# diepthihoang/mpboot

Hardware: AMD Instinct MI355X
Metric: Fitch site-ops/sec (taxa x patterns x SPR-evals/s) (higher is better)
Workload: dtype u32

## Files before the change

### mpboot_amd/csrc/engine.cpp

```cpp
#include "engine.hpp"
#include <cstdlib>
#include "../host/simd_util.hpp"

#include <sched.h>

#include <algorithm>
#include <atomic>
#include <thread>
#include <ctime>
#include <chrono>
#include <climits>
#include <cstdio>
#include <cstring>

namespace mpf {

static_assert(sizeof(PlanOp) == sizeof(NvOp) && offsetof(PlanOp, pad) == offsetof(NvOp, pad), "refresh_stage sizes the ops as NvOp");

static inline double now_ms()
{
  return std::chrono::duration<double, std::milli>(std::chrono::steady_clock::now().time_since_epoch()).count();
}
struct ScopedMs {
  double &acc, t0;
// ... 450 lines not shown
{
  if (m <= 1 || tip(q)) return 1;
  if (m == vis_dense_m_ && visits_filled_epoch_ == topo_epoch_) return vis_dense_[(size_t)slot(q)];
  const size_t key = (size_t)q * 16 + (size_t)m;
  if (nvis_epoch_[key] == topo_epoch_) return nvis_val_[key];
  const int v = 1 + count_visits(back_[nx(q)], m - 1) + count_visits(back_[nx(nx(q))], m - 1);
  nvis_val_[key] = v;
  nvis_epoch_[key] = topo_epoch_;
  return v;
}

bool Engine::dev_sched_usable() const
{
  return have_tree_ && all_invalid_ && dev_sched_ && !sankoff_ && ntips_ == n_ && n_ >= 4 && g_.vw == 1 && g_.nv_pipe && views_mode_ >= 1 &&
         nslots_ <= kSchedMaxSlots;
}

int Engine::schedule_views_dev(int sweep_maxtrav)
{
  ScopedMs timer(stats.host_views_ms_total);
  RefreshShape s;
  s.nops = 3 * (size_t)(n_ - 2);
  s.maxlev = -1;
  const size_t n_prune = sweep_maxtrav > 0 ? 2 * (size_t)n_ - 2 : 0;
  if (kids_host_.size() != nslots_) kids_host_.assign(nslots_, make_uint2(0u, 0u));
  for (int v = n_ + 1; v <= 2 * n_ - 2; v++) {
    const int r0 = 3 * v;
    const uint32_t s0 = slot(back_[r0]), s1 = slot(back_[r0 + 1]), s2 = slot(back_[r0 + 2]);
    uint2 *k = &kids_host_[slot(r0)];
    k[0] = make_uint2(s1, s2);
    k[1] = make_uint2(s2, s0);
    k[2] = make_uint2(s0, s1);
  }
  kids_list_.clear();
  const size_t no_ride[2] = {0, 0};
  const RefreshStage sg = refresh_stage(nslots_, s.nops, (size_t)n_ + 2, n_prune, 64, 0, no_ride);
  HIPCHK(h_kstage_.reserve(sg.ops_off));
  HIPCHK(d_vstage_.reserve(sg.total));
  std::memcpy(h_kstage_.p, kids_host_.data(), sg.kids_bytes);
  uint8_t *src = d_vstage_.p;
  SweepDescArgs sw;
  if (n_prune) {
    uint32_t *np = reinterpret_cast<uint32_t *>(h_kstage_.p + sg.nodep_off);
    for (size_t i = 0; i < n_prune; i++) np[i] = slot(nodep_[i + 1]);
    const size_t cap = 8 * n_prune;
    HIPCHK(d_walk_.reserve(cap));
// ... 1 lines not shown
    HIPCHK(h_dsw_.reserve(4 + cap));
    HIPCHK(d_prog_.reserve(scan_prog_bytes((int)cap)));
    HIPCHK(reserve_results(cap * 63));
    sw.nodep = np;
    sw.n_prune = (uint32_t)n_prune;
    sw.maxtrav = (uint32_t)sweep_maxtrav;
    sw.split_cands = (uint32_t)std::max(0, split_cands_);
    sw.desc = d_walk_.p;
    sw.parts = d_parts_.p;
    sw.hdr_host = h_dsw_.p;
    sw.part_node = h_dsw_.p + 4;
    sw.hdr_dev = reinterpret_cast<uint32_t *>(src + sg.nlev_off) + 8;
    __atomic_store_n(h_dsw_.p + 3, 0u, __ATOMIC_RELAXED);
    __atomic_store_n(h_dsw_.p + 2, 0u, __ATOMIC_RELAXED);
    walk_gen_++;
    n_walk_ = 0;
    walk_out_ = 0;
    sweep_cache_valid_ = false;
    s.sw = &sw;
  }
  kids_dirty_ = false;
  kids_upload_ = false;
  kids_dev_ready_ = true;
  HIPCHK(launch_sched(st_, reinterpret_cast<const uint2 *>(h_kstage_.p), (uint32_t)n_, (uint32_t)s.nops, reinterpret_cast<NvOp *>(src + sg.ops_off),
                      reinterpret_cast<int32_t *>(src + sg.lev_off), reinterpret_cast<int32_t *>(src + sg.nlev_off), sw, reinterpret_cast<uint2 *>(src)));
  int rc = launch_refresh(src, sg, s);
  if (rc) return rc;
  const std::vector<int> &all = plan_.all;
  plan_.whole_tree(start_);
  upd_order_.resize(s.nops);
  size_t at = 0;
  if (all.size() != s.nops) { set_error("refresh schedule: the tree is not complete"); return MPF_E_STATE; }
  for (size_t i = all.size(); i >= 3; i -= 3) upd_order_[at++] = all[i - 3];
  for (size_t i = 0; i < all.size(); i += 3) { upd_order_[at++] = all[i + 1]; upd_order_[at++] = all[i + 2]; }
  rc = commit_refresh(sg, s, true, 2, true);
  if (n_prune) dsw_sched_gen_ = sched_gen_;
  return rc;
}

int Engine::launch_refresh(const uint8_t *src, const RefreshStage &sg, const RefreshShape &s)
{
  const NvOp *dops = reinterpret_cast<const NvOp *>(src + sg.ops_off);
  const int32_t *dlo = reinterpret_cast<const int32_t *>(src + sg.lev_off);
  HIPCHK(d_cntp_.reserve((size_t)std::max(tiles_for(g_), tiles_for_levels(g_)) * nslots_));
  if (timing_ >= 2) HIPCHK(hipEventRecord(ev2_, st_));
  RefreshExtra x;
  if (s.maxlev < 0) x.n_lev_ptr = reinterpret_cast<const int32_t *>(src + sg.nlev_off);
  x.wm_only = refresh_wm_only(s.chains);
  if (!x.wm_only) { const int rc = ensure_rows(); if (rc) return rc; }
  x.rows = rows_ok_;
  cnt_on_host_ = s.fold_inside && want_host_results_;
  if (cnt_on_host_) x.cnt_host = h_cnt();
  for (int i = 0; i < 2; i++) ride_[i].dev = sg.ride_off[i] ? src + sg.ride_off[i] : nullptr;
  const bool zero = s.ride && zero_req_ptr_;
  x.zero_ptr = zeroed_ptr_ = zero ? zero_req_ptr_ : nullptr;
  x.zero_words = (uint32_t)(zeroed_words_ = zero ? zero_req_words_ : 0);
  if (s.sw && plan_ride_) {
    x.wp_kids = reinterpret_cast<const uint2 *>(src);
    x.wp_n = (uint32_t)n_;
    x.wp_desc = d_walk_.p;
    x.wp_hdr = s.sw->hdr_dev;
    x.wp_prog = d_prog_.p;
    x.wp_out = d_out();
    x.wp_max_parts = 8 * s.sw->n_prune;
  }
  uint32_t *const vec = vec_base();
  uint32_t *const done = s.fold_inside ? d_done_.p : nullptr;
  if (s.chains) {
    if (s.direct) {
      x.kid_upd = reinterpret_cast<const uint32_t *>(src + sg.upd_off);
      x.n_kid_upd = (int)(plan_.kid_upd.size() / 3);
      x.kids = reinterpret_cast<uint2 *>(d_vstage_.p);
    }
    HIPCHK(launch_newview_chains(st_, g_, vec, dops, dlo, plan_.ch_levels, (int)s.nops, d_cntp_.p, (uint32_t)nslots_, d_cnt(), done, x));
    stats.view_launches++;
  } else if (views_mode_ >= 1) {
    if (s.generic && nv_waves_ > 0) x.waves_hint = nv_waves_;
    else if (s.generic && nv_waves_ == 0 && s.maxlev > 0 && g_.vw == 1 && g_.nv_pipe && !sankoff_) {
      const long per_level = ((long)s.nops + s.maxlev - 1) / s.maxlev;
      const long need = (2 * per_level * newview_tile(g_) + 63) / 64;
      x.waves_hint = need <= 2 ? 2 : need <= 4 ? 4 : need <= 8 ? 8 : 16;
    }
    HIPCHK(launch_newview_levels(st_, g_, vec, dops, dlo, s.maxlev < 0 ? 1 : s.maxlev, d_cntp_.p, (uint32_t)nslots_, d_cnt(), done, x));
    if (x.wm_only) rows_ok_ = false;
    stats.view_launches++;
  } else {
    const int32_t *lo = reinterpret_cast<const int32_t *>(h_vstage_.p + sg.lev_off);
    for (int l = 0; l < s.maxlev; l++) {
      HIPCHK(launch_newview(st_, g_, vec, dops + lo[l], lo[l + 1] - lo[l], d_cntp_.p, (uint32_t)nslots_));
      stats.view_launches++;
    }
  }
  if (!s.fold_inside)
    HIPCHK(launch_cntsum(st_, g_, dops, (int)s.nops, d_cntp_.p, (uint32_t)nslots_, d_cnt(),
                         (views_mode_ >= 1 && !s.chains) ? tiles_for_levels(g_) : 0));
  if (timing_ >= 2) { HIPCHK(hipEventRecord(ev3_, st_)); view_events_pending_ = true; }
  cnt_copy_pending_ = true;
  return MPF_OK;
}

int Engine::commit_refresh(const RefreshStage &sg, const RefreshShape &s, bool full, int made, bool cacheable)
{
  const bool both = views_mode_ >= 1 && !sankoff_ && g_.vw == 1 && g_.shoff != 0 && (s.chains || g_.nv_pipe);
  if (!both) shadow_ok_ = false;
  for (int r : upd_order_) valid_[r] = 1;
  all_invalid_ = false;
  if (full) { n_invalid_ = 0; views_valid_ = true; }
  else if (n_invalid_ > 0) {
    n_invalid_ -= (long)s.nops;
    if (n_invalid_ <= 0) {
      n_invalid_ = 0;
      views_valid_ = true;
      if (check_counts_)
        for (size_t r = 3 * ((size_t)n_ + 1); r < back_.size(); r++)
          if (back_[r] >= 0 && !valid_[r]) { set_error("view bookkeeping: invalid vector left behind"); return MPF_E_STATE; }
    }
  }
  pending_scores_ = true;
  if (made) {
    sched_cache_valid_ = (plan_cache_ & 2) && cacheable;
    sched_gen_++;
    sched_on_dev_ = made == 2;
    sc_stage_ = sg;
    if (sched_cache_valid_) { sc_maxlev_ = s.maxlev; sc_order_ = upd_order_; }
  }
  stats.newview_ops += s.nops;
  if (s.maxlev >= 0) dbg_levels_ += (uint64_t)(s.chains ? plan_.ch_levels : s.maxlev);
  stats.algorithmic_bytes += (uint64_t)s.nops * 3u * (uint64_t)g_.S * (uint64_t)Wref_ * 4u;
  return MPF_OK;
}

int Engine::schedule_views(const std::vector<int> *roots)
{
  if (!have_tree_) { set_error("no tree set"); return MPF_E_STATE; }
  ScopedMs timer(stats.host_views_ms_total);
  RefreshShape s;
  if (!roots && all_invalid_ && sched_cache_valid_ && !kids_dirty_ && !sankoff_) {
    s.nops = sc_order_.size();
    s.maxlev = sc_maxlev_;
    const int rc = launch_refresh(d_vstage_.p, sc_stage_, s);
    if (rc) return rc;
    upd_order_ = sc_order_;
    return commit_refresh(sc_stage_, s, true, 0, false);
  }
  if (!roots && dev_sched_usable()) return schedule_views_dev(0);
  const bool full = !roots;
  if (full) { plan_.whole_tree(start_); roots = &plan_.all; }
  const bool from_scratch = full && all_invalid_;
  plan_.close(*roots, from_scratch);
  if (kids_host_.size() != nslots_) kids_host_.assign(nslots_, make_uint2(0u, 0u));
  s.generic = true;
  const size_t nops = s.nops = plan_.order.size();
  s.maxlev = plan_.maxlev;
  s.chains = views_mode_ == 2 && !sankoff_ && nops > 0 && (long)nops <= chain_max_ops_ && g_.S * g_.vw <= 8;
  s.direct = s.chains && kids_dev_ready_ && (kids_dirty_ ? roots->size() + nops : kids_list_.size()) <= 4096;
  s.fold_inside = views_mode_ >= 1 && !sankoff_ && nops <= 512;
  s.ride = !sankoff_ && nops > 0 && views_mode_ >= 1;
  const auto slot_of = [this](int r) { return slot(r); };
  if (plan_.topo_delta(reinterpret_cast<uint32_t *>(kids_host_.data()), kids_list_, kids_dirty_, *roots, full, s.direct, slot_of))
// ... 759 lines not shown
    dsw_valid_ = false;
    rc = schedule_views_dev(mt);
  }
  if (rc) return rc;
  ScopedMs timer(stats.host_scan_ms_total);
  if (!warm) {
    if (!wait_host_flag(h_dsw_.p + 3)) HIPCHK(hipStreamSynchronize(st_));
    dsw_parts_ = h_dsw_.p[0];
    dsw_out_ = h_dsw_.p[1];
    dsw_walk_gen_ = walk_gen_;
    std::copy(key, key + 4, dsw_key_);
    dsw_valid_ = true;
  }
  const size_t nd = dsw_parts_, nout = dsw_out_;
  uint32_t best = UINT_MAX;
  if (nd > 0) {
    HIPCHK(d_ncand_.reserve(nd));
    HIPCHK(reserve_results(nout));
    HIPCHK(d_prog_.reserve(scan_prog_bytes((int)nd)));
    HIPCHK(h_pmin_.reserve(nd + 1));
    if (warm) HIPCHK(hipMemsetAsync(d_out(), 0, clear_words(nout) * sizeof(uint32_t), st_));
    if (timing_) HIPCHK(hipEventRecord(ev0_, st_));
    if (!warm) {
      if (!plan_ride_) HIPCHK(launch_walk_plan(st_, d_kids(), n_, d_walk_.p, (int)nd, d_prog_.p, d_out(), (uint32_t)clear_words(nout)));
      prog_gen_ = walk_gen_;
      parts_gen_ = walk_gen_;
      n_parts_dev_ = nd;
    }
    const bool wm = shadow_ok_ && scan_shadow_ && scan_prog_word_major(g_);
    HIPCHK(launch_scan_prog(st_, g_, wm ? vec_base() : vec_rows(), d_walk_.p, (int)nd, d_prog_.p, d_out(), d_ncand_.p, nullptr, (uint32_t)nout, d_done_.p + 8, nullptr,
                            wm));
    stats.plan_launches++;
    if (timing_) HIPCHK(hipEventRecord(ev1_, st_));
    __atomic_store_n(h_pmin_.p + nd, 0u, __ATOMIC_RELAXED);
    HIPCHK(launch_part_min(st_, d_out(), d_parts_.p, (int)nd, h_pmin_.p, d_cnt(), cnt_copy_pending_ ? h_cnt() : nullptr, (uint32_t)nslots_,
                           d_done_.p + 24));
    cnt_copy_pending_ = false;
    if (!wait_host_flag(h_pmin_.p + nd)) HIPCHK(hipStreamSynchronize(st_));
    float ms = 0;
    if (timing_ && hipEventElapsedTime(&ms, ev0_, ev1_) == hipSuccess) { stats.last_scan_kernel_ms = ms; stats.scan_kernel_ms_total += ms; }
    if (plan_event_pending_) {
      if (hipEventElapsedTime(&ms, ev4_, ev0_) == hipSuccess) stats.plan_kernel_ms_total += ms;
      plan_event_pending_ = false;
    }
    stats.scan_launches++;
  } else {
    if (cnt_copy_pending_) {
// ... 132 lines not shown
  long sum = 0;
  int site = 0;
  for (int k = 0; k < P_ && site < n_sites; k++) {
    if (first_site_[(size_t)k] < 0) continue;
    for (int w = 0; w < wgt_[(size_t)k] && site < n_sites; w++) { site_pars[site++] = ptn[(size_t)k]; sum += ptn[(size_t)k]; }
  }
  for (; site < n_sites; site++) site_pars[site] = 0;
  if (total) *total = (int32_t)sum;
  return MPF_OK;
}

int Engine::set_option(const std::string &key, int64_t v)
{
  if (key == "scan_batch") { if (v < 1) return MPF_E_INVALID; scan_batch_ = (int)v; return MPF_OK; }
  if (key == "words_per_lane") {
    if (sankoff_ && v != 1) { set_error("words_per_lane: weighted mode uses one pattern per lane"); return MPF_E_INVALID; }
    if (!(v == 1 || v == 2 || v == 4) || (g_.S == 20 && v == 4)) { set_error("words_per_lane: 1|2|4 (protein: 1|2)"); return MPF_E_INVALID; }
    if (g_.S >= 20) return MPF_OK;
    g_.vw = (int)v;
    return MPF_OK;
  }
  if (key == "dev_sched") { dev_sched_ = v != 0; sched_cache_valid_ = false; dsw_valid_ = false; return MPF_OK; }
  if (key == "dev_plan") { dev_plan_ = v != 0; plan_ride_ = !(v & 2); dsw_valid_ = false; return MPF_OK; }
  if (key == "refresh_wm") { refresh_wm_ = v != 0; return MPF_OK; }
  if (key == "scan_shadow") { scan_shadow_ = v != 0; return MPF_OK; }
  if (key == "reduce") { g_.reduce = v ? 1 : 0; return MPF_OK; }
  if (key == "xcd_map") { g_.map = v ? 1 : 0; return MPF_OK; }
  if (key == "scan_mode") { scan_mode_ = v ? 1 : 0; return MPF_OK; }
  if (key == "views_pipe") { g_.nv_pipe = v != 0; sched_cache_valid_ = false; return MPF_OK; }
  if (key == "views_tile") {
    if (v != 32 && v != 16 && v != 8 && v != 4 && v != 0) { set_error("views_tile: 32, 16, 8 or 4 words (0: chosen from the row length)"); return MPF_E_INVALID; }
    g_.nv_tile = (int)v;
    sched_cache_valid_ = false;
    return MPF_OK;
  }
  if (key == "views_mode") { views_mode_ = v < 0 ? 0 : v > 2 ? 2 : (int)v; sched_cache_valid_ = false; return MPF_OK; }
  if (key == "host_poll") { host_poll_ = v ? 1 : 0; return MPF_OK; }
  if (key == "ufb_fast") { ufb_fast_ = v ? 1 : 0; return MPF_OK; }
  if (key == "ufb_quiet") { ufb_quiet_ = v ? 1 : 0; return MPF_OK; }
  if (key == "deep_scratch_kwords") {
    if (v < 1 || v > (1 << 22)) { set_error("deep_scratch_kwords: 1 .. 4194304"); return MPF_E_INVALID; }
    deep_scratch_words_ = (size_t)v << 10; d_deep_.release(); g_.deep_scratch = nullptr; g_.deep_scratch_words = 0;
    return MPF_OK;
  }
  if (key == "grow_device") { grow_device_ = v ? 1 : 0; return MPF_OK; }
  if (key == "grow_tile") { if (v != 0 && v != 1 && v != 2 && v != 4 && v != 8 && v != -1) { set_error("grow_tile: 0 (word-major copy where there is one, else fitted), -1 (fitted quad tiles), 1, 2, 4 or 8"); return MPF_E_INVALID; } grow_vw_ = (int)v; return MPF_OK; }
// ... 60 lines not shown
  return MPF_E_INVALID;
}

int Engine::scan_trace(uint64_t *out, uint64_t cap, uint64_t *n)
{
  if (climb_trace_) {
    *n = cd_.h_trace.size() / 2;
    if (cap >= *n && *n) std::memcpy(out, cd_.h_trace.data(), cd_.h_trace.size() * sizeof(uint32_t));
    return MPF_OK;
  }
  *n = trace_words_;
  if (!trace_words_ || cap < trace_words_) return MPF_OK;
  activate();
  HIPCHK(hipMemcpy(out, d_trace_.p, trace_words_ * sizeof(unsigned long long), hipMemcpyDeviceToHost));
  return MPF_OK;
}

int Engine::get_option(const std::string &key, int64_t *v) const
{
  if (key == "scan_prog") *v = scan_prog_;
  else if (key == "prog_min_descs") *v = prog_min_descs_;
  else if (key == "refresh_wm") *v = refresh_wm_ ? 1 : 0;
  else if (key == "refresh_wm_active") *v = (refresh_wm_ && !sankoff_ && g_.S == 4 && g_.shoff != 0) ? 1 : 0;
  else if (key == "rows_ok") *v = rows_ok_ ? 1 : 0;
  else if (key == "ensure_rows_launches") *v = (int64_t)ensure_rows_launches_;
  else if (key == "scan_batch") *v = scan_batch_;
  else if (key == "words_per_lane") *v = g_.vw;
  else if (key == "kernel_states") *v = g_.S;
  else if (key == "reduce") *v = g_.reduce;
  else if (key == "xcd_map") *v = g_.map;
  else if (key == "scan_mode") *v = scan_mode_;
  else if (key == "views_mode") *v = views_mode_;
  else if (key == "views_pipe") *v = g_.nv_pipe;
  else if (key == "views_tile") *v = g_.nv_tile;
  else if (key == "plan_cache") *v = plan_cache_;
  else if (key == "sched_levels" || key == "sched_ticks" || key == "sched_desc_ticks") {
    int32_t w[16] = {0};
    if (sched_on_dev_ && d_vstage_.p) { (void)hipStreamSynchronize(st_); (void)hipMemcpy(w, d_vstage_.p + sc_stage_.nlev_off, 64, hipMemcpyDeviceToHost); }
    *v = w[key == "sched_levels" ? 0 : key == "sched_ticks" ? 1 : 2];
  }
  else if (key == "split_below") *v = split_below_;
  else if (key == "split_cands") *v = split_cands_;
  else if (key == "chain_max_ops") *v = chain_max_ops_;
  else if (key == "timing") *v = timing_;
  else if (key == "ufb_fast") *v = ufb_fast_;
  else if (key == "ufb_quiet") *v = ufb_quiet_;
// ... 80 lines not shown
```

### mpboot_amd/csrc/engine.hpp

```cpp
#pragma once
#include <hip/hip_runtime.h>

#include <algorithm>
#include <cmath>
#include <chrono>
#include <cstdint>
#include <functional>
#include <map>
#include <unordered_map>
#include <memory>
#include <climits>
#include <set>
#include <string>
#include <utility>
#include <vector>

#include "../../include/mpfitch.h"
#include "../host/rng.hpp"
#include "../host/ufb_books.hpp"
#include "../host/list_tree.hpp"
#include "../host/split_sets.hpp"
#include "../host/refresh_plan.hpp"
#include "../host/many_shape.hpp"
#include "climb.hpp"
// ... 202 lines not shown
  int P() const { return P_; }
  int S() const { return sref_; }
  int Wref() const { return Wref_; }
  int Wp() const { return g_.Wp; }
  int n_informative() const { return ninf_; }
  const std::vector<int32_t> &informative() const { return inf_; }

  int set_tree(const int32_t *back);
  void get_tree(int32_t *back) const;
  void reset_node_order();
  void node_rectifier();

  int score_tree(uint32_t *score);
  int pattern_scores(uint16_t *ptn, int32_t *total);
  int site_scores(int32_t *site_pars, int n_sites, int32_t *total);
  int update_views();
  int tree_length(uint32_t *len);
  void invalidate_all();
  void invalidate_vectors();
  void invalidate_node(int node);
  int schedule_views(const std::vector<int> *roots);
  bool dev_sched_usable() const;
  int schedule_views_dev(int sweep_maxtrav);
  struct RefreshShape { size_t nops = 0; int maxlev = 0; bool chains = false, direct = false, fold_inside = false, generic = false, ride = false;
                        const SweepDescArgs *sw = nullptr; };
  int launch_refresh(const uint8_t *src, const RefreshStage &sg, const RefreshShape &s);
  int commit_refresh(const RefreshStage &sg, const RefreshShape &s, bool full, int made, bool cacheable);
  int sweep_scan_dev(int maxtrav, uint64_t *n_tests, uint32_t *min_mp);
  void finish_views();
  void collect_scan_roots(int p, int mintrav, int maxtrav, std::vector<int> &roots) const;

  int plan_scan(int rec, int mintrav, int maxtrav, ScanPlan &plan);
  int run_scans(std::vector<ScanPlan> &plans, std::vector<uint32_t> &out_host);
  int plan_walk(int rec, int mintrav, int maxtrav, ScanPlan &plan, bool split);
  int run_walks(std::vector<ScanPlan> &plans, const uint32_t **out_host);
  int run_walks_finish(std::vector<ScanPlan> &plans, const uint32_t **out_host);
  static bool wait_host_flag(const uint32_t *flag);
  struct WaitScope { WaitScope(); ~WaitScope(); };
  static void wait_pause();
  int scan_batch(std::vector<ScanPlan> &plans, const int *recs, int count, int mintrav, int maxtrav, const uint32_t **out);
  int candidate_record(const ScanPlan &plan, size_t c);
  void enumerate_side(int x, int mintrav, int maxtrav, std::vector<int32_t> &q) const { enumerate_side(back_, x, mintrav, maxtrav, q); }
  void enumerate_side(const std::vector<int32_t> &bk, int x, int mintrav, int maxtrav, std::vector<int32_t> &q) const { books::enumerate_side(n_, bk, x, mintrav, maxtrav, q); }
  int spr_scan(int rec, int mintrav, int maxtrav, std::vector<int32_t> &q, std::vector<uint32_t> &mp, int &n_p);
  int sweep_scan(int mintrav, int maxtrav, uint64_t *n_tests, uint32_t *min_mp);
  int sweep_costs(int mintrav, int maxtrav, uint64_t cap, uint32_t *mp, uint64_t *offsets, uint64_t *n_tests);
  int node_order(int32_t *recs);
// ... 421 lines not shown
  int scan_mode_ = 1;
  int scan_prog_ = 1, prog_min_descs_ = 256;
  DevBuf<uint8_t> d_prog_;
  int plan_cache_ = 7;
  bool sched_cache_valid_ = false;
  RefreshStage sc_stage_ = {};
  int sc_maxlev_ = 0;
  bool dev_sched_ = true;
  bool dev_plan_ = true;
  PinBuf<uint8_t> h_kstage_;
  PinBuf<uint32_t> h_dsw_;
  bool dsw_valid_ = false;
  uint64_t dsw_walk_gen_ = 0;
  uint64_t sched_gen_ = 0, dsw_sched_gen_ = ~0ull;
  int dsw_key_[4] = {0, 0, 0, 0};
  uint32_t dsw_parts_ = 0, dsw_out_ = 0;
  bool sched_on_dev_ = false;
  bool shadow_ok_ = false;
  bool scan_shadow_ = true;
  bool rows_ok_ = true;
  bool refresh_wm_ = true;
  uint64_t ensure_rows_launches_ = 0;
  bool plan_ride_ = true;
  std::vector<int> sc_order_;
  bool sweep_cache_valid_ = false, walk_dev_reuse_ = false;
  uint64_t walk_gen_ = 0, sweep_cache_gen_ = 0;
  uint64_t prog_gen_ = ~0ull;
  size_t sweep_cache_nwalk_ = 0;
  uint32_t sweep_cache_out_ = 0;
  int sweep_cache_key_[6] = {0, 0, 0, 0, 0, 0};
  std::vector<int> sweep_cache_recs_;
  int scan_trace_ = 0;
  DevBuf<unsigned long long> d_trace_;
  size_t trace_words_ = 0;
  std::vector<uint32_t> out_scratch_;
  std::vector<ScanPlan> sweep_plans_;
  std::vector<uint32_t> sc_keep_mp_;
  std::vector<uint64_t> sc_keep_off_;
  uint64_t sc_keep_key_[4] = {0, 0, 0, 0}, pack_gen_ = 0;
  bool sc_keep_valid_ = false;
  std::vector<int32_t> nvis_val_, nvis_epoch_;
  int32_t topo_epoch_ = 1;
  int count_visits(int q, int m);
  void fill_visit_counts(int maxm);
  int32_t visits_filled_epoch_ = 0;
  std::vector<int32_t> vis_dense_, vis_a_;
// ... 50 lines not shown
```

### mpboot_amd/csrc/kernels.hip

```cpp
#include "kernels.hpp"
#include <cstdlib>

namespace mpf {


__device__ __forceinline__ uint32_t wave_sum_dpp(uint32_t v)
{
  v += (uint32_t)__builtin_amdgcn_update_dpp(0, (int)v, 0xB1, 0xF, 0xF, false);
  v += (uint32_t)__builtin_amdgcn_update_dpp(0, (int)v, 0x4E, 0xF, 0xF, false);
  v += (uint32_t)__builtin_amdgcn_update_dpp(0, (int)v, 0x141, 0xF, 0xF, false);
  v += (uint32_t)__builtin_amdgcn_update_dpp(0, (int)v, 0x140, 0xF, 0xF, false);
  v += (uint32_t)__builtin_amdgcn_update_dpp(0, (int)v, 0x142, 0xA, 0xF, false);
  v += (uint32_t)__builtin_amdgcn_update_dpp(0, (int)v, 0x143, 0xC, 0xF, false);
  return v;
}

template <int TW>
__device__ __forceinline__ uint32_t group_sum(uint32_t v)
{
  v += (uint32_t)__builtin_amdgcn_update_dpp(0, (int)v, 0xB1, 0xF, 0xF, false);
  v += (uint32_t)__builtin_amdgcn_update_dpp(0, (int)v, 0x4E, 0xF, 0xF, false);
  if constexpr (TW >= 8) v += (uint32_t)__builtin_amdgcn_update_dpp(0, (int)v, 0x141, 0xF, 0xF, false);
  if constexpr (TW >= 16) v += (uint32_t)__builtin_amdgcn_update_dpp(0, (int)v, 0x140, 0xF, 0xF, false);
  if constexpr (TW == 32) v += (uint32_t)__shfl_xor((int)v, 16, 32);
// ... 222 lines not shown
  const int w0 = lane_word<VW>(tile, lane, Wp, valid);
  Tile<S, VW> a, b, c;
  load_tile<S, VW>(a, vec, o.a, Wp, w0);
  load_tile<S, VW>(b, vec, o.b, Wp, w0);
  uint32_t cost = fitch<S, VW>(c, a, b);
  if (valid) store_tile<S, VW>(c, vec, o.dst, Wp, w0);
  cost = valid ? cost : 0u;
  const uint32_t tot = wave_total<RED>(cost);
  if (lane == 0) cntp[(size_t)tile * nslots + o.dst] = tot;
}

template <int S, int VW, int RED>
__global__ __launch_bounds__(256) void k_newview(uint32_t *__restrict__ vec, const NvOp *__restrict__ ops, int n_ops,
                                                 uint32_t *__restrict__ cntp, uint32_t nslots, int Wp, int tiles)
{
  const int lane = threadIdx.x & 63;
  int gw = blockIdx.x * (blockDim.x >> 6) + (threadIdx.x >> 6);
  gw = __builtin_amdgcn_readfirstlane(gw);
  if (gw >= n_ops * tiles) return;
  const int op = gw / tiles, tile = gw - op * tiles;
  newview_one<S, VW, RED>(vec, ops[op], cntp, nslots, Wp, tile, lane);
}

__device__ __forceinline__ void fold_counts(const NvOp *__restrict__ ops, int n_ops, const uint32_t *__restrict__ cntp,
                                            uint32_t nslots, int tiles, uint32_t *__restrict__ cnt, int tid, int nthreads,
                                            uint32_t *__restrict__ cnt_host = nullptr)
{
  const int l32 = tid & 31, grp = tid >> 5, ngrp = nthreads >> 5;
  for (int i = grp; i < n_ops; i += 2 * ngrp) {
    const int j = i + ngrp < n_ops ? i + ngrp : i;
    const uint32_t d0 = ops[i].dst, d1 = ops[j].dst;
    uint32_t s0 = 0, s1 = 0;
    for (int t = l32; t < tiles; t += 32) {
      s0 += __builtin_nontemporal_load(cntp + (size_t)t * nslots + d0);
      s1 += __builtin_nontemporal_load(cntp + (size_t)t * nslots + d1);
    }
#pragma unroll
    for (int m = 16; m >= 1; m >>= 1) {
      s0 += (uint32_t)__shfl_xor((int)s0, m, 32);
      s1 += (uint32_t)__shfl_xor((int)s1, m, 32);
    }
    if (l32 == 0) {
      cnt[d0] = s0;
      if (j != i) cnt[d1] = s1;
      if (cnt_host) {
        cnt_host[d0] = s0;
        if (j != i) cnt_host[d1] = s1;
      }
    }
  }
}

template <int S, int VW, int RED>
__global__ __launch_bounds__(1024) void k_newview_wg(uint32_t *__restrict__ vec, const NvOp *__restrict__ ops,
                                                     const int32_t *__restrict__ lev_off, int n_lev,
                                                     uint32_t *__restrict__ cntp, uint32_t nslots, int Wp,
                                                     uint32_t *__restrict__ cnt, uint32_t *__restrict__ done,
                                                     RefreshExtra x)
{
  __shared__ int s_last;
  const int lane = threadIdx.x & 63;
  const int wave = __builtin_amdgcn_readfirstlane((int)(threadIdx.x >> 6));
  const int nw = (int)(blockDim.x >> 6);
  const int tile = blockIdx.x;
  bool valid;
  const int w0 = lane_word<VW>(tile, lane, Wp, valid);
  for (uint32_t i = blockIdx.x * blockDim.x + threadIdx.x; i < x.zero_words; i += gridDim.x * blockDim.x) x.zero_ptr[i] = 0u;
  for (int l = 0; l < n_lev; l++) {
    const int b = lev_off[l], e = lev_off[l + 1];
    int i = b + wave;
    for (; i + nw < e; i += 2 * nw) {
      const NvOp o0 = ops[i], o1 = ops[i + nw];
      Tile<S, VW> a0, b0, a1, b1, c0, c1;
// ... 475 lines not shown
  if (per <= 2u) return launch(int_c<2>());
  if (per <= 3u) return launch(int_c<3>());
  if (per <= 4u) return launch(int_c<4>());
  if (per <= 6u) return launch(int_c<6>());
  if (per <= 8u) return launch(int_c<8>());
  return launch(int_c<16>());
}

__global__ __launch_bounds__(256) void k_cntsum(const NvOp *__restrict__ ops, int n_ops, const uint32_t *__restrict__ cntp, uint32_t nslots,
                                                int tiles, uint32_t *__restrict__ cnt, uint32_t *__restrict__ cnt_host)
{
  const int l32 = threadIdx.x & 31;
  const int i = (int)(blockIdx.x * (blockDim.x >> 5) + (threadIdx.x >> 5));
  if (i >= n_ops) return;
  const uint32_t dst = ops[i].dst;
  uint32_t s = 0;
  for (int t = l32; t < tiles; t += 32) s += cntp[(size_t)t * nslots + dst];
#pragma unroll
  for (int m = 16; m >= 1; m >>= 1) s += (uint32_t)__shfl_xor((int)s, m, 32);
  if (l32 == 0) {
    cnt[dst] = s;
    if (cnt_host) cnt_host[dst] = s;
  }
}


template <int S, int VW, int RED, bool WM = false>
__global__ __launch_bounds__(256) void k_evaluate(const uint32_t *__restrict__ vec, const EvOp *__restrict__ ops,
                                                  int n_ops, uint32_t *__restrict__ out, int Wp, int tiles)
{
  const int lane = threadIdx.x & 63;
  int gw = blockIdx.x * (blockDim.x >> 6) + (threadIdx.x >> 6);
  gw = __builtin_amdgcn_readfirstlane(gw);
  if (gw >= n_ops * tiles) return;
  const int op = gw / tiles, tile = gw - op * tiles;
  const EvOp o = ops[op];
  bool valid;
  const int w0 = lane_word<VW>(tile, lane, Wp, valid);
  Tile<S, VW> a, b;
  if constexpr (WM) {
    static_assert(S == 4 && VW == 1, "word-major copy: DNA, one word per lane");
    load_tile_wm(a, vec, o.a, Wp, w0);
    load_tile_wm(b, vec, o.b, Wp, w0);
  } else {
    load_tile<S, VW>(a, vec, o.a, Wp, w0);
    load_tile<S, VW>(b, vec, o.b, Wp, w0);
// ... 2088 lines not shown
```

### mpboot_amd/csrc/kernels.hpp

```cpp
#pragma once
#include <hip/hip_runtime.h>
#include <stdint.h>
#include <atomic>
#include <type_traits>

#include "../host/list_tree.hpp"

namespace mpf {

struct NvOp { uint32_t dst, a, b, pad; };

struct EvOp { uint32_t a, b, out, pad; };

struct ScanOp { uint32_t own, sib, meta, out; };
struct ScanHdr { uint32_t op_begin, op_end, s_slot, pad ; };

enum { SCAN_CHAIN = 0, SCAN_ROOT = 1, SCAN_JOIN = 2, SCAN_EVAL = 3 };

struct WalkDesc { uint32_t s_cid, xa_cid, xb_cid, trav ,
                  out_base, pad0, pad1, pad2; };
constexpr int kWalkMaxDepth = 8;
constexpr int kMaxDepth = 12;
constexpr int scan_reg_depth(int S, bool sankoff) { return sankoff ? (S != 4 ? 6 : kMaxDepth) : (S >= 32 ? 6 : kMaxDepth); }

// ... 79 lines not shown
                            const uint32_t *tip_slots);
hipError_t launch_newview(hipStream_t st, const Geometry &g, uint32_t *vec, const NvOp *ops, int n_ops, uint32_t *cntp,
                          uint32_t nslots);
struct RefreshExtra { const uint32_t *kid_upd = nullptr; int n_kid_upd = 0; uint2 *kids = nullptr; uint32_t *zero_ptr = nullptr; uint32_t zero_words = 0;
                      uint32_t *cnt_host = nullptr;
                      const int32_t *n_lev_ptr = nullptr;
                      const uint2 *wp_kids = nullptr; uint32_t wp_n = 0; const WalkDesc *wp_desc = nullptr; const uint32_t *wp_hdr = nullptr ;
                      void *wp_prog = nullptr; uint32_t *wp_out = nullptr; uint32_t wp_max_parts = 0;
                      uint32_t *shadow = nullptr;
                      int wm_only = 0, rows = 0;
                      int waves_hint = 0;  };
constexpr uint32_t kSchedMaxSlots = 16384;
struct SweepDescArgs {
  const uint32_t *nodep = nullptr;
  uint32_t n_prune = 0, maxtrav = 0, split_cands = 0;
  WalkDesc *desc = nullptr;
  uint2 *parts = nullptr;
  uint32_t *part_node = nullptr;
  uint32_t *hdr_host = nullptr;
  uint32_t *hdr_dev = nullptr;
};
hipError_t launch_sched(hipStream_t st, const uint2 *kids, uint32_t n_taxa, uint32_t n_ops, NvOp *ops, int32_t *lev_off, int32_t *n_lev,
                        const SweepDescArgs &sw = SweepDescArgs(), uint2 *kids_copy = nullptr);
hipError_t launch_newview_levels(hipStream_t st, const Geometry &g, uint32_t *vec, const NvOp *ops, const int32_t *lev_off,
                                 int n_lev, uint32_t *cntp, uint32_t nslots, uint32_t *cnt, uint32_t *done,
                                 const RefreshExtra &x = RefreshExtra());
hipError_t launch_newview_chains(hipStream_t st, const Geometry &g, uint32_t *vec, const NvOp *ops, const int32_t *wl_off,
                                 int n_lev, int n_ops, uint32_t *cntp, uint32_t nslots, uint32_t *cnt, uint32_t *done,
                                 const RefreshExtra &x);
hipError_t launch_part_min(hipStream_t st, const uint32_t *out, const uint2 *parts, int n_parts, uint32_t *pmin,
                           const uint32_t *cnt = nullptr, uint32_t *cnt_host = nullptr, uint32_t n_cnt = 0, uint32_t *done = nullptr);
hipError_t launch_cntsum(hipStream_t st, const Geometry &g, const NvOp *ops, int n_ops, const uint32_t *cntp,
                         uint32_t nslots, uint32_t *cnt, int tiles = 0 ,
                         uint32_t *cnt_host = nullptr );
int tiles_for(const Geometry &g);
int newview_tile(const Geometry &g);
int tiles_for_levels(const Geometry &g);
hipError_t launch_evaluate(hipStream_t st, const Geometry &g, const uint32_t *vec, const EvOp *ops, int n_ops,
                           uint32_t *out, bool word_major = false);
hipError_t launch_rows_from_wm(hipStream_t st, const Geometry &g, uint32_t *vec, const uint32_t *slots, int n_slots);
struct NniDesc { uint32_t a, b, c0, c1; };
hipError_t launch_nni_eval(hipStream_t st, const Geometry &g, const uint32_t *vec, const NniDesc *desc, int n_br,
                           unsigned long long *out, int vw, bool word_major);
hipError_t launch_nni_eval_masks(hipStream_t st, const Geometry &g, const uint32_t *vec, const NniDesc *desc, int n_br,
                                 unsigned long long *out, int vw, bool word_major, uint32_t *plane0, uint32_t *plane1);
hipError_t launch_snk_nni_eval(hipStream_t st, const Geometry &g, const uint32_t *vec, const NniDesc *desc, int n_br,
// ... 46 lines not shown
```

Baseline: 18080000 billion.

## Fuse level scheduling into the full-tree newview kernel for self-scheduled refresh

A new kernel builds the level lists itself. Each block derives the next level's ready ops in LDS while it computes Fitch for the current level, so the separate launch_sched kernel and the device ops/level arrays are no longer needed on the main path. A small kids-copy kernel replaces the scheduling launch. The count fold runs inside the kernel for small trees, and otherwise in a slot-indexed cntsum that can also carry the walk-plan work. Each block redundantly recomputes the schedule in 1024-thread blocks with large LDS, which may limit occupancy, and an optional extra block writes out the ops list for caching.

```diff
diff --git a/mpboot_amd/csrc/engine.cpp b/mpboot_amd/csrc/engine.cpp
--- a/mpboot_amd/csrc/engine.cpp
+++ b/mpboot_amd/csrc/engine.cpp
@@ -496,6 +496,9 @@
   RefreshShape s;
   s.nops = 3 * (size_t)(n_ - 2);
   s.maxlev = -1;
+  s.self = refresh_self_sched_ && newview_self_supported(g_, (uint32_t)n_, (uint32_t)s.nops);
+  s.fold_inside = s.self && s.nops <= 512;
+  self_active_ = s.self;
   const size_t n_prune = sweep_maxtrav > 0 ? 2 * (size_t)n_ - 2 : 0;
   if (kids_host_.size() != nslots_) kids_host_.assign(nslots_, make_uint2(0u, 0u));
   for (int v = n_ + 1; v <= 2 * n_ - 2; v++) {
@@ -543,8 +546,11 @@
   kids_dirty_ = false;
   kids_upload_ = false;
   kids_dev_ready_ = true;
-  HIPCHK(launch_sched(st_, reinterpret_cast<const uint2 *>(h_kstage_.p), (uint32_t)n_, (uint32_t)s.nops, reinterpret_cast<NvOp *>(src + sg.ops_off),
-                      reinterpret_cast<int32_t *>(src + sg.lev_off), reinterpret_cast<int32_t *>(src + sg.nlev_off), sw, reinterpret_cast<uint2 *>(src)));
+  if (s.self)
+    HIPCHK(launch_kids_copy(st_, reinterpret_cast<const uint2 *>(h_kstage_.p), reinterpret_cast<uint2 *>(src), (uint32_t)n_, (uint32_t)s.nops));
+  else
+    HIPCHK(launch_sched(st_, reinterpret_cast<const uint2 *>(h_kstage_.p), (uint32_t)n_, (uint32_t)s.nops, reinterpret_cast<NvOp *>(src + sg.ops_off),
+                        reinterpret_cast<int32_t *>(src + sg.lev_off), reinterpret_cast<int32_t *>(src + sg.nlev_off), sw, reinterpret_cast<uint2 *>(src)));
   int rc = launch_refresh(src, sg, s);
   if (rc) return rc;
   const std::vector<int> &all = plan_.all;
@@ -576,7 +582,8 @@
   const bool zero = s.ride && zero_req_ptr_;
   x.zero_ptr = zeroed_ptr_ = zero ? zero_req_ptr_ : nullptr;
   x.zero_words = (uint32_t)(zeroed_words_ = zero ? zero_req_words_ : 0);
-  if (s.sw && plan_ride_) {
+  plan_rode_ = s.sw && plan_ride_ && !(s.self && s.fold_inside);
+  if (plan_rode_) {
     x.wp_kids = reinterpret_cast<const uint2 *>(src);
     x.wp_n = (uint32_t)n_;
     x.wp_desc = d_walk_.p;
@@ -594,6 +601,14 @@
       x.kids = reinterpret_cast<uint2 *>(d_vstage_.p);
     }
     HIPCHK(launch_newview_chains(st_, g_, vec, dops, dlo, plan_.ch_levels, (int)s.nops, d_cntp_.p, (uint32_t)nslots_, d_cnt(), done, x));
+    stats.view_launches++;
+  } else if (s.self) {
+    HIPCHK(launch_newview_self(st_, g_, vec, reinterpret_cast<const uint2 *>(src), (uint32_t)n_, (uint32_t)s.nops, d_cntp_.p, (uint32_t)nslots_, d_cnt(), done,
+                               reinterpret_cast<int32_t *>(d_vstage_.p + sg.nlev_off), reinterpret_cast<const uint2 *>(h_kstage_.p),
+                               s.sw ? *s.sw : SweepDescArgs(), x,
+                               (plan_cache_ & 2) ? reinterpret_cast<NvOp *>(d_vstage_.p + sg.ops_off) : nullptr,
+                               (plan_cache_ & 2) ? reinterpret_cast<int32_t *>(d_vstage_.p + sg.lev_off) : nullptr));
+    if (x.wm_only) rows_ok_ = false;
     stats.view_launches++;
   } else if (views_mode_ >= 1) {
     if (s.generic && nv_waves_ > 0) x.waves_hint = nv_waves_;
@@ -612,7 +627,9 @@
       stats.view_launches++;
     }
   }
-  if (!s.fold_inside)
+  if (s.self) {
+    if (!s.fold_inside) HIPCHK(launch_cntsum_slots(st_, (uint32_t)n_, (int)s.nops, d_cntp_.p, (uint32_t)nslots_, d_cnt(), tiles_for_levels(g_), x));
+  } else if (!s.fold_inside)
     HIPCHK(launch_cntsum(st_, g_, dops, (int)s.nops, d_cntp_.p, (uint32_t)nslots_, d_cnt(),
                          (views_mode_ >= 1 && !s.chains) ? tiles_for_levels(g_) : 0));
   if (timing_ >= 2) { HIPCHK(hipEventRecord(ev3_, st_)); view_events_pending_ = true; }
@@ -656,6 +673,7 @@
   if (!have_tree_) { set_error("no tree set"); return MPF_E_STATE; }
   ScopedMs timer(stats.host_views_ms_total);
   RefreshShape s;
+  if (all_invalid_) self_active_ = false;
   if (!roots && all_invalid_ && sched_cache_valid_ && !kids_dirty_ && !sankoff_) {
     s.nops = sc_order_.size();
     s.maxlev = sc_maxlev_;
@@ -1461,7 +1479,7 @@
     if (warm) HIPCHK(hipMemsetAsync(d_out(), 0, clear_words(nout) * sizeof(uint32_t), st_));
     if (timing_) HIPCHK(hipEventRecord(ev0_, st_));
     if (!warm) {
-      if (!plan_ride_) HIPCHK(launch_walk_plan(st_, d_kids(), n_, d_walk_.p, (int)nd, d_prog_.p, d_out(), (uint32_t)clear_words(nout)));
+      if (!plan_rode_) HIPCHK(launch_walk_plan(st_, d_kids(), n_, d_walk_.p, (int)nd, d_prog_.p, d_out(), (uint32_t)clear_words(nout)));
       prog_gen_ = walk_gen_;
       parts_gen_ = walk_gen_;
       n_parts_dev_ = nd;
@@ -1640,6 +1658,7 @@
   }
   if (key == "dev_sched") { dev_sched_ = v != 0; sched_cache_valid_ = false; dsw_valid_ = false; return MPF_OK; }
   if (key == "dev_plan") { dev_plan_ = v != 0; plan_ride_ = !(v & 2); dsw_valid_ = false; return MPF_OK; }
+  if (key == "refresh_self_sched") { refresh_self_sched_ = v != 0; sched_cache_valid_ = false; dsw_valid_ = false; return MPF_OK; }
   if (key == "refresh_wm") { refresh_wm_ = v != 0; return MPF_OK; }
   if (key == "scan_shadow") { scan_shadow_ = v != 0; return MPF_OK; }
   if (key == "reduce") { g_.reduce = v ? 1 : 0; return MPF_OK; }
@@ -1746,6 +1765,8 @@
   else if (key == "prog_min_descs") *v = prog_min_descs_;
   else if (key == "refresh_wm") *v = refresh_wm_ ? 1 : 0;
   else if (key == "refresh_wm_active") *v = (refresh_wm_ && !sankoff_ && g_.S == 4 && g_.shoff != 0) ? 1 : 0;
+  else if (key == "refresh_self_sched") *v = refresh_self_sched_ ? 1 : 0;
+  else if (key == "refresh_self_sched_active") *v = self_active_ ? 1 : 0;
   else if (key == "rows_ok") *v = rows_ok_ ? 1 : 0;
   else if (key == "ensure_rows_launches") *v = (int64_t)ensure_rows_launches_;
   else if (key == "scan_batch") *v = scan_batch_;
diff --git a/mpboot_amd/csrc/engine.hpp b/mpboot_amd/csrc/engine.hpp
--- a/mpboot_amd/csrc/engine.hpp
+++ b/mpboot_amd/csrc/engine.hpp
@@ -248,7 +248,8 @@
   int schedule_views(const std::vector<int> *roots);
   bool dev_sched_usable() const;
   int schedule_views_dev(int sweep_maxtrav);
-  struct RefreshShape { size_t nops = 0; int maxlev = 0; bool chains = false, direct = false, fold_inside = false, generic = false, ride = false;
+  struct RefreshShape { size_t nops = 0; int maxlev = 0; bool chains = false, direct = false, fold_inside = false, generic = false, ride = false,
+                             self = false;
                         const SweepDescArgs *sw = nullptr; };
   int launch_refresh(const uint8_t *src, const RefreshStage &sg, const RefreshShape &s);
   int commit_refresh(const RefreshStage &sg, const RefreshShape &s, bool full, int made, bool cacheable);
@@ -716,6 +717,9 @@
   bool refresh_wm_ = true;
   uint64_t ensure_rows_launches_ = 0;
   bool plan_ride_ = true;
+  bool plan_rode_ = false;
+  bool refresh_self_sched_ = true;
+  bool self_active_ = false;
   std::vector<int> sc_order_;
   bool sweep_cache_valid_ = false, walk_dev_reuse_ = false;
   uint64_t walk_gen_ = 0, sweep_cache_gen_ = 0;
diff --git a/mpboot_amd/csrc/kernels.hip b/mpboot_amd/csrc/kernels.hip
--- a/mpboot_amd/csrc/kernels.hip
+++ b/mpboot_amd/csrc/kernels.hip
@@ -268,14 +268,15 @@
   newview_one<S, VW, RED>(vec, ops[op], cntp, nslots, Wp, tile, lane);
 }
 
-__device__ __forceinline__ void fold_counts(const NvOp *__restrict__ ops, int n_ops, const uint32_t *__restrict__ cntp,
-                                            uint32_t nslots, int tiles, uint32_t *__restrict__ cnt, int tid, int nthreads,
-                                            uint32_t *__restrict__ cnt_host = nullptr)
+template <class DstOf>
+__device__ __forceinline__ void fold_counts_of(DstOf dst_of, int n_ops, const uint32_t *__restrict__ cntp,
+                                               uint32_t nslots, int tiles, uint32_t *__restrict__ cnt, int tid, int nthreads,
+                                               uint32_t *__restrict__ cnt_host)
 {
   const int l32 = tid & 31, grp = tid >> 5, ngrp = nthreads >> 5;
   for (int i = grp; i < n_ops; i += 2 * ngrp) {
     const int j = i + ngrp < n_ops ? i + ngrp : i;
-    const uint32_t d0 = ops[i].dst, d1 = ops[j].dst;
+    const uint32_t d0 = dst_of(i), d1 = dst_of(j);
     uint32_t s0 = 0, s1 = 0;
     for (int t = l32; t < tiles; t += 32) {
       s0 += __builtin_nontemporal_load(cntp + (size_t)t * nslots + d0);
@@ -295,6 +296,12 @@
       }
     }
   }
+}
+__device__ __forceinline__ void fold_counts(const NvOp *__restrict__ ops, int n_ops, const uint32_t *__restrict__ cntp,
+                                            uint32_t nslots, int tiles, uint32_t *__restrict__ cnt, int tid, int nthreads,
+                                            uint32_t *__restrict__ cnt_host = nullptr)
+{
+  fold_counts_of([ops](int i) { return ops[i].dst; }, n_ops, cntp, nslots, tiles, cnt, tid, nthreads, cnt_host);
 }
 
 template <int S, int VW, int RED>
@@ -816,6 +823,280 @@
     cnt[dst] = s;
     if (cnt_host) cnt_host[dst] = s;
   }
+}
+
+static size_t self_sched_lds_bytes(uint32_t n, uint32_t n_ops, bool desc)
+{
+  const size_t ns = (size_t)n + n_ops;
+  const size_t a = (size_t)n_ops * 4 + ((ns * 2 + 15) & ~(size_t)15) + (((size_t)n_ops * 2 + 15) & ~(size_t)15);
+  return desc ? std::max(a, sched_lds_bytes(n, (uint32_t)ns, true)) : a;
+}
+
+__global__ __launch_bounds__(256) void k_kids_copy(const uint2 *__restrict__ src, uint2 *__restrict__ dst, uint32_t first, uint32_t count)
+{
+  const uint32_t i = blockIdx.x * blockDim.x + threadIdx.x;
+  if (i < count) dst[first + i] = src[first + i];
+}
+
+template <int S, int TW, bool WM = false>
+__global__ __launch_bounds__(1024) void k_newview_self(uint32_t *__restrict__ vec, const uint2 *__restrict__ kids, uint32_t n, uint32_t n_ops,
+                                                       uint32_t *__restrict__ cntp, uint32_t nslots, int Wp, uint32_t *__restrict__ cnt,
+                                                       uint32_t *__restrict__ done, int32_t *__restrict__ diag,
+                                                       const uint2 *__restrict__ kids_host, SweepDescArgs sw, RefreshExtra x,
+                                                       NvOp *__restrict__ ops_out, int32_t *__restrict__ lev_off_out)
+{
+  static_assert(!WM || S == 4, "word-major copy: DNA");
+  constexpr int OPI = 64 / TW;
+  constexpr int kRegRecs = S == 4 ? 4 : S <= 20 ? 1 : 0;
+  constexpr int kRegArr = kRegRecs ? kRegRecs : 1;
+  constexpr bool EARLY = S == 4;
+  extern __shared__ __attribute__((aligned(16))) uint8_t s_mem[];
+  __shared__ uint32_t s_c[3], s_wsum[32];
+  __shared__ int s_last;
+  const int nt = Wp / TW;
+  const bool lister = ops_out != nullptr && blockIdx.x == gridDim.x - 1u;
+  if ((int)blockIdx.x >= nt && !lister) {
+    const unsigned long long t_begin = __builtin_amdgcn_s_memrealtime();
+    sweep_desc_block(kids_host, n, n_ops, sw, s_mem, s_wsum);
+    if (threadIdx.x == 0u) diag[2] = (int32_t)(__builtin_amdgcn_s_memrealtime() - t_begin);
+    return;
+  }
+  const uint32_t tid = threadIdx.x, ns = n + n_ops;
+  const int lane = (int)(tid & 63u);
+  const int wave = __builtin_amdgcn_readfirstlane((int)(tid >> 6));
+  constexpr int nw = 16;
+  const bool timed = blockIdx.x == 0u;
+  const unsigned long long t_begin = timed ? __builtin_amdgcn_s_memrealtime() : 0ull;
+  uint32_t *s_k = reinterpret_cast<uint32_t *>(s_mem);
+  uint16_t *s_lev = reinterpret_cast<uint16_t *>(s_mem + (size_t)n_ops * 4);
+  uint16_t *s_list = reinterpret_cast<uint16_t *>(s_mem + (size_t)n_ops * 4 + (((size_t)ns * 2 + 15) & ~(size_t)15));
+  auto packed = [&](uint32_t k) { const uint2 v = kids[n + k]; return min(v.x, ns - 1u) | (min(v.y, ns - 1u) << 16); };
+  uint32_t kk[kRegArr];
+#pragma unroll
+  for (int j = 0; j < kRegRecs; j++) {
+    const uint32_t k = tid + 1024u * (uint32_t)j;
+    kk[j] = k < n_ops ? packed(k) : 0u;
+    if (k < n_ops) s_k[k] = kk[j];
+  }
+  for (uint32_t k = tid + 1024u * (uint32_t)kRegRecs; k < n_ops; k += 1024u) s_k[k] = packed(k);
+  for (uint32_t c = tid; c < ns; c += 1024u) s_lev[c] = c < n ? (uint16_t)0 : (uint16_t)0xFFFFu;
+  if (tid < 3u) s_c[tid] = 0u;
+  __syncthreads();
+  auto list_next = [&](uint32_t l, uint32_t e) {
+    uint32_t *const ctr = &s_c[(l + 1u) % 3u];
+    const unsigned long long below = (1ull << lane) - 1ull;
+    bool rdy[kRegArr];
+    uint32_t pre[kRegArr], tot = 0;
+#pragma unroll
+    for (int j = 0; j < kRegRecs; j++) {
+      rdy[j] = false;
+      if (__ballot(kk[j] != 0u) != 0ull) {
+        const uint32_t la = s_lev[kk[j] & 0xFFFFu], lb = s_lev[kk[j] >> 16];
+        rdy[j] = kk[j] != 0u && la <= l && lb <= l;
+        if (la <= l) kk[j] &= 0xFFFF0000u;
+        if (lb <= l) kk[j] &= 0x0000FFFFu;
+      }
+    }
+#pragma unroll
+    for (int j = 0; j < kRegRecs; j++) {
+      const unsigned long long m = __ballot(rdy[j]);
+      pre[j] = tot + (uint32_t)__builtin_popcountll(m & below);
+      tot += (uint32_t)__builtin_popcountll(m);
+    }
+    if (tot) {
+      uint32_t at = 0;
+      if (lane == 0) at = atomicAdd(ctr, tot);
+      at = e + (uint32_t)__builtin_amdgcn_readfirstlane((int)at);
+#pragma unroll
+      for (int j = 0; j < kRegRecs; j++)
+        if (rdy[j]) {
+          const uint32_t c = n + tid + 1024u * (uint32_t)j;
+          s_list[at + pre[j]] = (uint16_t)c;
+          s_lev[c] = (uint16_t)(l + 1u);
+          kk[j] = 0u;
+        }
+    }
+    for (uint32_t k0 = 1024u * (uint32_t)kRegRecs + (tid & ~63u); k0 < n_ops; k0 += 1024u) {
+      const uint32_t k = k0 + (uint32_t)lane;
+      bool r = false;
+      if (k < n_ops && s_lev[n + k] == 0xFFFFu) {
+        const uint32_t v = s_k[k];
+        r = s_lev[v & 0xFFFFu] <= l && s_lev[v >> 16] <= l;
+      }
+      const unsigned long long m = __ballot(r);
+      if (m != 0ull) {
+        uint32_t at = 0;
+        if (lane == 0) at = atomicAdd(ctr, (uint32_t)__builtin_popcountll(m));
+        at = e + (uint32_t)__builtin_amdgcn_readfirstlane((int)at);
+        if (r) {
+          s_list[at + (uint32_t)__builtin_popcountll(m & below)] = (uint16_t)(n + k);
+          s_lev[n + k] = (uint16_t)(l + 1u);
+        }
+      }
+    }
+  };
+  list_next(0u, 0u);
+  __syncthreads();
+  const uint32_t ticks = timed ? (uint32_t)(__builtin_amdgcn_s_memrealtime() - t_begin) : 0u;
+  const int xcd = (int)(blockIdx.x & 7u), q8 = nt >> 3, r8 = nt & 7;
+  const int tile = xcd * q8 + min(xcd, r8) + (int)(blockIdx.x >> 3);
+  const int sub = lane / TW;
+  const int w0 = tile * TW + (lane % TW);
+  const int step = OPI * nw;
+  auto op_at = [&](int i) {
+    const uint32_t c = s_list[i], v = s_k[c - n];
+    return NvOp{c, v & 0xFFFFu, v >> 16, 0u};
+  };
+  auto ld = [&](Tile<S, 1> &t, uint32_t slot) {
+    if constexpr (WM) load_tile_wm(t, x.shadow, slot, Wp, w0);
+    else load_tile<S, 1>(t, vec, slot, Wp, w0);
+  };
+  uint32_t l = 1, b = 0;
+  for (;; l++) {
+    const uint32_t in_level = s_c[l % 3u];
+    if (tid == 0u) s_c[(l + 2u) % 3u] = 0u;
+    if (in_level == 0u) break;
+    const int e = (int)(b + in_level);
+    int ib = (int)b + OPI * wave;
+    const bool mine = !lister && ib < e;
+    if (lister && tid == 0u) lev_off_out[l - 1u] = (int32_t)b;
+    NvOp o = {0u, 0u, 0u, 0u}, o1 = o;
+    Tile<S, 1> ta, tb;
+    auto first = [&]() {
+      o = op_at(min(ib + sub, e - 1));
+      o1 = op_at(min(ib + step + sub, e - 1));
+      ld(ta, o.a);
+      ld(tb, o.b);
+    };
+    if constexpr (EARLY)
+      if (mine) first();
+    list_next(l, (uint32_t)e);
+    if (mine) {
+      if constexpr (!EARLY) first();
+      for (; ib < e; ib += step) {
+        const NvOp o2 = op_at(min(ib + 2 * step + sub, e - 1));
+        Tile<S, 1> na, nb, tc;
+        ld(na, o1.a);
+        ld(nb, o1.b);
+        const uint32_t k = fitch<S, 1>(tc, ta, tb);
+        if constexpr (WM) store_tile_wm(tc, x.shadow, o.dst, Wp, w0);
+        else store_tile<S, 1>(tc, vec, o.dst, Wp, w0);
+        if constexpr (S == 4 && !WM)
+          if (x.shadow) *reinterpret_cast<uint4 *>(x.shadow + ((size_t)o.dst * (size_t)Wp + (size_t)w0) * 4) = make_uint4(tc.v[0][0], tc.v[1][0], tc.v[2][0], tc.v[3][0]);
+        cntp[(size_t)tile * nslots + o.dst] = group_sum<TW>(k);
+        ta = na; tb = nb; o = o1; o1 = o2;
+      }
+    }
+    __syncthreads();
+    b = (uint32_t)e;
+  }
+  if (timed && tid == 0u) { diag[0] = (int32_t)(l - 1u); diag[1] = (int32_t)ticks; }
+  if (lister) {
+    for (uint32_t i = tid; i < b; i += 1024u) {
+      const NvOp o = op_at((int)i);
+      const uint32_t k = o.dst - n;
+      ops_out[i] = NvOp{o.dst, o.a, o.b, 3u * (n + 1u + k / 3u) + k % 3u};
+    }
+    if (tid == 0u) lev_off_out[l - 1u] = (int32_t)b;
+    return;
+  }
+  if (!done) return;
+  if (tid == 0u) {
+    __builtin_amdgcn_fence(__ATOMIC_RELEASE, "agent");
+    const uint32_t ticket = __hip_atomic_fetch_add(done, 1u, __ATOMIC_RELAXED, __HIP_MEMORY_SCOPE_AGENT);
+    s_last = ticket == (uint32_t)nt - 1u;
+  }
+  __syncthreads();
+  if (s_last) {
+    __builtin_amdgcn_fence(__ATOMIC_ACQUIRE, "agent");
+    fold_counts_of([n](int i) { return n + (uint32_t)i; }, (int)n_ops, cntp, nslots, nt, cnt, (int)tid, 1024, x.cnt_host);
+    if (tid == 0u) __hip_atomic_store(done, 0u, __ATOMIC_RELAXED, __HIP_MEMORY_SCOPE_AGENT);
+  }
+}
+
+bool newview_self_supported(const Geometry &g, uint32_t n_taxa, uint32_t n_ops)
+{
+  if (g.S > 20 && newview_tile(g) == 32) return false;
+  return !g.sankoff && g.vw == 1 && g.nv_pipe && n_taxa >= 3u && n_ops >= 1u && n_taxa + n_ops <= kSchedMaxSlots;
+}
+
+hipError_t launch_kids_copy(hipStream_t st, const uint2 *src, uint2 *dst, uint32_t first, uint32_t count)
+{
+  if (!count) return hipSuccess;
+  hipLaunchKernelGGL(k_kids_copy, dim3((count + 255u) / 256u), dim3(256), 0, st, src, dst, first, count);
+  return hipGetLastError();
+}
+
+hipError_t launch_newview_self(hipStream_t st, const Geometry &g, uint32_t *vec, const uint2 *kids, uint32_t n_taxa, uint32_t n_ops,
+                               uint32_t *cntp, uint32_t nslots, uint32_t *cnt, uint32_t *done, int32_t *diag, const uint2 *kids_host,
+                               const SweepDescArgs &sw, const RefreshExtra &x, NvOp *ops_out, int32_t *lev_off_out)
+{
+  if (!newview_self_supported(g, n_taxa, n_ops)) return hipErrorInvalidValue;
+  if ((ops_out != nullptr) != (lev_off_out != nullptr)) return hipErrorInvalidValue;
+  if (sw.nodep && (!kids_host || sw.maxtrav < 1u || sw.maxtrav > 6u)) return hipErrorInvalidValue;
+  if (x.wm_only && !(g.S == 4 && g.shoff)) return hipErrorInvalidValue;
+  RefreshExtra xs = x;
+  if (g.shoff && g.S == 4) xs.shadow = vec + g.shoff;
+  const int tw = newview_tile(g);
+  const size_t lds = self_sched_lds_bytes(n_taxa, n_ops, sw.nodep != nullptr);
+  dim3 grid((unsigned)(g.Wp / tw) + (sw.nodep ? 1u : 0u) + (ops_out ? 1u : 0u)), block(1024);
+  hipError_t err = hipSuccess;
+  dispatch_states(g.S, [&](auto S) {
+    auto launch = [&](auto TW, auto WM) {
+      err = lds_opt_in<k_newview_self<S, TW, WM>>(160 * 1024);
+      if (err != hipSuccess) return;
+      hipLaunchKernelGGL((k_newview_self<S, TW, WM>), grid, block, lds, st, vec, kids, n_taxa, n_ops, cntp, nslots, g.Wp, cnt, done, diag,
+                         kids_host, sw, xs, ops_out, lev_off_out);
+    };
+    auto by_tile = [&](auto WM) {
+      if (tw == 32) {
+        if constexpr (S <= 20) launch(int_c<32>(), WM);
+      } else if (tw == 16) launch(int_c<16>(), WM); else if (tw == 8) launch(int_c<8>(), WM); else launch(int_c<4>(), WM);
+    };
+    if constexpr (S == 4) {
+      if (xs.wm_only) { by_tile(bool_c<true>()); return; }
+    }
+    by_tile(bool_c<false>());
+  });
+  return err != hipSuccess ? err : hipGetLastError();
+}
+
+__global__ __launch_bounds__(256) void k_cntsum_slots(uint32_t first, int n_ops, const uint32_t *__restrict__ cntp, uint32_t nslots, int tiles,
+                                                      uint32_t *__restrict__ cnt, uint32_t *__restrict__ cnt_host, uint32_t plan_blocks,
+                                                      RefreshExtra x)
+{
+  if (blockIdx.x < plan_blocks) {
+    const uint32_t n_parts = x.wp_hdr[0], n_out = x.wp_hdr[1];
+    const uint32_t nw = blockDim.x >> 6, wave = threadIdx.x >> 6;
+    const uint32_t zw = ((n_out ? n_out : 1u) + 1u + 63u) & ~63u;
+    for (uint32_t i = blockIdx.x * blockDim.x + threadIdx.x; i < zw; i += plan_blocks * blockDim.x) x.wp_out[i] = 0u;
+    for (uint32_t item = blockIdx.x * nw + wave; item < 2u * n_parts; item += plan_blocks * nw)
+      walk_plan_item(x.wp_kids, x.wp_n, x.wp_desc, (int)n_parts, static_cast<ProgEnt *>(x.wp_prog), 0xFFFFFFFFu, (int)item, (int)(threadIdx.x & 63u));
+    return;
+  }
+  const int l32 = threadIdx.x & 31;
+  const int i = (int)((blockIdx.x - plan_blocks) * (blockDim.x >> 5) + (threadIdx.x >> 5));
+  if (i >= n_ops) return;
+  const uint32_t dst = first + (uint32_t)i;
+  uint32_t s = 0;
+  for (int t = l32; t < tiles; t += 32) s += cntp[(size_t)t * nslots + dst];
+#pragma unroll
+  for (int m = 16; m >= 1; m >>= 1) s += (uint32_t)__shfl_xor((int)s, m, 32);
+  if (l32 == 0) {
+    cnt[dst] = s;
+    if (cnt_host) cnt_host[dst] = s;
+  }
+}
+
+hipError_t launch_cntsum_slots(hipStream_t st, uint32_t first, int n_ops, const uint32_t *cntp, uint32_t nslots, uint32_t *cnt, int tiles,
+                               const RefreshExtra &x)
+{
+  const unsigned plan_blocks = x.wp_desc ? std::min(2048u, (2u * x.wp_max_parts + 15u) / 16u) : 0u;
+  const unsigned fold_blocks = n_ops > 0 ? (unsigned)((n_ops + 7) / 8) : 0u;
+  if (plan_blocks + fold_blocks == 0u) return hipSuccess;
+  hipLaunchKernelGGL(k_cntsum_slots, dim3(plan_blocks + fold_blocks), dim3(256), 0, st, first, n_ops, cntp, nslots, tiles, cnt, x.cnt_host,
+                     plan_blocks, x);
+  return hipGetLastError();
 }
 
 
diff --git a/mpboot_amd/csrc/kernels.hpp b/mpboot_amd/csrc/kernels.hpp
--- a/mpboot_amd/csrc/kernels.hpp
+++ b/mpboot_amd/csrc/kernels.hpp
@@ -125,6 +125,14 @@
 };
 hipError_t launch_sched(hipStream_t st, const uint2 *kids, uint32_t n_taxa, uint32_t n_ops, NvOp *ops, int32_t *lev_off, int32_t *n_lev,
                         const SweepDescArgs &sw = SweepDescArgs(), uint2 *kids_copy = nullptr);
+bool newview_self_supported(const Geometry &g, uint32_t n_taxa, uint32_t n_ops);
+hipError_t launch_newview_self(hipStream_t st, const Geometry &g, uint32_t *vec, const uint2 *kids, uint32_t n_taxa, uint32_t n_ops,
+                               uint32_t *cntp, uint32_t nslots, uint32_t *cnt, uint32_t *done, int32_t *diag, const uint2 *kids_host,
+                               const SweepDescArgs &sw, const RefreshExtra &x,
+                               NvOp *ops_out = nullptr, int32_t *lev_off_out = nullptr);
+hipError_t launch_kids_copy(hipStream_t st, const uint2 *src, uint2 *dst, uint32_t first, uint32_t count);
+hipError_t launch_cntsum_slots(hipStream_t st, uint32_t first, int n_ops, const uint32_t *cntp, uint32_t nslots, uint32_t *cnt, int tiles,
+                               const RefreshExtra &x);
 hipError_t launch_newview_levels(hipStream_t st, const Geometry &g, uint32_t *vec, const NvOp *ops, const int32_t *lev_off,
                                  int n_lev, uint32_t *cntp, uint32_t nslots, uint32_t *cnt, uint32_t *done,
                                  const RefreshExtra &x = RefreshExtra());
```

New measurement: 19080000 billion, median of 6. 1.06x the previous value.
